# indrajeetadityaroy9/vit-bias-aware-structural-distillation

Measured on AMD Instinct MI355X. Metric: images/sec BASD train step, DeiT-T student / ViT-B teacher bs=256, higher is better.
Workload: dtype bf16

## Files before the change

### vit-bias-aware-structural-distillation_amd/csrc/attention.hip

```cpp
#include "basd_frag.h"

namespace basd {

__device__ __forceinline__ unsigned short f32_to_bf16_rne(float f) {
  unsigned int u = __float_as_uint(f);
  u += 0x7fffu + ((u >> 16) & 1u);
  return (unsigned short)(u >> 16);
}

template <int CTRL> __device__ __forceinline__ float at_dpp_add(float v) {
  return v + __int_as_float(__builtin_amdgcn_update_dpp(0, __float_as_int(v), CTRL, 0xF, 0xF, true));
}

template <int NKT, int AT_HD, bool QMEAN = false>
__global__ __launch_bounds__(256) __attribute__((amdgpu_waves_per_eu(2, 2))) void attention_fwd_kernel(const unsigned short* __restrict__ qkv, int T, int H,
                                                            float scale, unsigned short* __restrict__ out,
                                                            float* __restrict__ importance, float* __restrict__ lse) {
  constexpr int NKS = (NKT + 1) / 2;
  constexpr int KROWS = 32 * NKS;
  constexpr int NDS = (AT_HD + 31) / 32;
  constexpr int NDT = AT_HD / 16;
  constexpr int NCH = AT_HD / 8;
  constexpr int NCHP = NDS * 4;
  constexpr int AT_LD = NDS * 32 + 8;
  extern __shared__ __align__(16) unsigned short sm[];
  unsigned short* Ks = sm;
  unsigned short* Vs = Ks + KROWS * AT_LD;
  unsigned short* Os = Vs + KROWS * AT_LD;
  const int tid = threadIdx.x, lane = tid & 63, wave = tid >> 6;
  const int li = lane & 15, g = lane >> 4;
  const int b = blockIdx.x / H, h = blockIdx.x - b * H;
  const size_t row = (size_t)3 * H * AT_HD;
  const unsigned short* base = qkv + (size_t)b * T * row + (size_t)h * AT_HD;

  constexpr int NLD = (KROWS * NCHP + 255) / 256;
  uint4 kreg[NLD], vreg[NLD];
#pragma unroll
  for (int i = 0; i < NLD; ++i) {
    const int idx = tid + 256 * i;
    const int r = idx / NCHP, c8 = idx - r * NCHP;
    kreg[i] = make_uint4(0, 0, 0, 0);
    vreg[i] = make_uint4(0, 0, 0, 0);
    if (r < T && c8 < NCH) {
      const unsigned short* p = base + (size_t)r * row + c8 * 8;
      kreg[i] = *reinterpret_cast<const uint4*>(p + (size_t)H * AT_HD);
      vreg[i] = *reinterpret_cast<const uint4*>(p + (size_t)2 * H * AT_HD);
    }
  }
#pragma unroll
  for (int i = 0; i < NLD; ++i) {
    const int idx = tid + 256 * i;
    const int r = idx / NCHP, c8 = idx - r * NCHP;
    if (idx < KROWS * NCHP) {
      *reinterpret_cast<uint4*>(Ks + r * AT_LD + c8 * 8) = kreg[i];
      *reinterpret_cast<uint4*>(Vs + r * AT_LD + c8 * 8) = vreg[i];
    }
  }
  __syncthreads();

  const float sl2 = scale * 1.4426950408889634f;
  const int nqt = (T + 15) >> 4;
  const int full_tiles = T >> 4;
  unsigned short* Ow = Os + wave * 16 * AT_LD;
  auto load_q = [&](int qt_, uint4 (&dst)[NDS]) {
#pragma unroll
    for (int ks = 0; ks < NDS; ++ks) {
      dst[ks] = make_uint4(0, 0, 0, 0);
      if (qt_ < nqt && qt_ * 16 + li < T && 32 * ks + 8 * g < AT_HD)
        dst[ks] = *reinterpret_cast<const uint4*>(base + (size_t)(qt_ * 16 + li) * row + 32 * ks + 8 * g);
    }
  };
  uint4 qnext[NDS];
  load_q(wave, qnext);
  float csum[QMEAN ? NKT : 1][4];
#pragma unroll
  for (int kt = 0; kt < (QMEAN ? NKT : 1); ++kt)
#pragma unroll
    for (int r = 0; r < 4; ++r) csum[kt][r] = 0.f;
  for (int qt = wave; qt < nqt; qt += 4) {
    const int q0 = qt * 16;
    bf16x8 qf[NDS];
#pragma unroll
    for (int ks = 0; ks < NDS; ++ks) qf[ks] = *reinterpret_cast<bf16x8*>(&qnext[ks]);
    load_q(qt + 4, qnext);
    f32x4 s[NKT];
#pragma unroll
    for (int kt = 0; kt < NKT; ++kt) {
      f32x4 acc = {0.f, 0.f, 0.f, 0.f};
#pragma unroll
      for (int ks = 0; ks < NDS; ++ks) {
        const uint4 kk = *reinterpret_cast<const uint4*>(Ks + (16 * kt + li) * AT_LD + 32 * ks + 8 * g);
        acc = __builtin_amdgcn_mfma_f32_16x16x32_bf16(*reinterpret_cast<const bf16x8*>(&kk), qf[ks], acc, 0, 0, 0);
      }
      s[kt] = acc;
      if ((kt & 3) == 3) __builtin_amdgcn_sched_barrier(0);
    }
    if (!QMEAN && importance != nullptr && qt == 0) {
      float lr[NKT][4];
      float tmx = -3.0e38f;
#pragma unroll
      for (int kt = 0; kt < NKT; ++kt)
#pragma unroll
        for (int r = 0; r < 4; r += 2) {
          const unsigned int w = pack_bf16(s[kt][r], s[kt][r + 1]);
          lr[kt][r] = __uint_as_float(w << 16) * scale;
          lr[kt][r + 1] = __uint_as_float(w & 0xffff0000u) * scale;
          if (kt >= full_tiles) {
            if (16 * kt + 4 * g + r >= T) lr[kt][r] = -3.0e38f;
            if (16 * kt + 4 * g + r + 1 >= T) lr[kt][r + 1] = -3.0e38f;
          }
          tmx = fmaxf(tmx, fmaxf(lr[kt][r], lr[kt][r + 1]));
        }
      tmx = fmaxf(tmx, __shfl_xor(tmx, 16, 64));
      tmx = fmaxf(tmx, __shfl_xor(tmx, 32, 64));
      float tsum = 0.f;
#pragma unroll
      for (int kt = 0; kt < NKT; ++kt)
#pragma unroll
        for (int r = 0; r < 4; ++r) {
          lr[kt][r] = __builtin_amdgcn_exp2f((lr[kt][r] - tmx) * 1.4426950408889634f);
          tsum += lr[kt][r];
        }
      tsum += __shfl_xor(tsum, 16, 64);
      tsum += __shfl_xor(tsum, 32, 64);
      if (li == 0) {
        const float tinv = 1.f / (tsum * (float)H);
#pragma unroll
        for (int kt = 0; kt < NKT; ++kt)
#pragma unroll
          for (int r = 0; r < 4; ++r) {
            const int key = 16 * kt + 4 * g + r;
            if (key >= 1 && (kt < full_tiles || key < T))
              importance[((size_t)b * H + h) * (T - 1) + key - 1] = lr[kt][r] * tinv;
          }
      }
    }
    float mx = -3.0e38f;
#pragma unroll
    for (int kt = 0; kt < NKT; ++kt)
#pragma unroll
      for (int r = 0; r < 4; ++r) {
        if (kt >= full_tiles && 16 * kt + 4 * g + r >= T) s[kt][r] = -3.0e38f;
        mx = fmaxf(mx, s[kt][r]);
      }
    mx = fmaxf(mx, __shfl_xor(mx, 16, 64));
    mx = fmaxf(mx, __shfl_xor(mx, 32, 64));
    float sum = 0.f;
#pragma unroll
    for (int kt = 0; kt < NKT; ++kt)
#pragma unroll
      for (int r = 0; r < 4; ++r) {
        const float p = __builtin_amdgcn_exp2f((s[kt][r] - mx) * sl2);
        s[kt][r] = p;
        sum += p;
      }
    sum += __shfl_xor(sum, 16, 64);
    sum += __shfl_xor(sum, 32, 64);
    const float inv = 1.f / sum;
    if constexpr (QMEAN) {
      const float qinv = (q0 + li < T) ? inv : 0.f;
#pragma unroll
      for (int kt = 0; kt < NKT; ++kt)
#pragma unroll
        for (int r = 0; r < 4; ++r) csum[kt][r] = fmaf(s[kt][r], qinv, csum[kt][r]);
    }
    if (lse != nullptr && g == 0 && q0 + li < T) lse[((size_t)b * H + h) * T + q0 + li] = fmaf(mx, scale, __logf(sum));
    f32x4 o[NDT];
#pragma unroll
    for (int dt = 0; dt < NDT; ++dt) o[dt] = (f32x4){0.f, 0.f, 0.f, 0.f};
#pragma unroll
    for (int ks = 0; ks < NKS; ++ks) {
      const int K1 = (2 * ks + 1 < NKT) ? 2 * ks + 1 : 0;
      uint4 pw;
      pw.x = pack_bf16(s[2 * ks][0] * inv, s[2 * ks][1] * inv);
      pw.y = pack_bf16(s[2 * ks][2] * inv, s[2 * ks][3] * inv);
      pw.z = (2 * ks + 1 < NKT) ? pack_bf16(s[K1][0] * inv, s[K1][1] * inv) : 0u;
      pw.w = (2 * ks + 1 < NKT) ? pack_bf16(s[K1][2] * inv, s[K1][3] * inv) : 0u;
      const bf16x8 pa = *reinterpret_cast<const bf16x8*>(&pw);
      const int qq = li >> 2, pp = li & 3;
#pragma unroll
      for (int dt = 0; dt < NDT; ++dt) {
        const unsigned short* a0 = Vs + (32 * ks + 4 * g + qq) * AT_LD + 16 * dt + 4 * pp;
        const v4s lo = __builtin_amdgcn_ds_read_tr16_b64_v4i16((lds_v4s*)a0);
        const v4s hi = __builtin_amdgcn_ds_read_tr16_b64_v4i16((lds_v4s*)(a0 + 16 * AT_LD));
        const bf16x8 vb = {lo[0], lo[1], lo[2], lo[3], hi[0], hi[1], hi[2], hi[3]};
        o[dt] = __builtin_amdgcn_mfma_f32_16x16x32_bf16(pa, vb, o[dt], 0, 0, 0);
      }
    }
#pragma unroll
    for (int dt = 0; dt < NDT; ++dt)
#pragma unroll
      for (int r = 0; r < 4; r += 2) {
        const unsigned int w = pack_bf16(o[dt][r], o[dt][r + 1]);
        Ow[(4 * g + r) * AT_LD + 16 * dt + li] = (unsigned short)(w & 0xffffu);
        Ow[(4 * g + r + 1) * AT_LD + 16 * dt + li] = (unsigned short)(w >> 16);
      }
    __builtin_amdgcn_s_waitcnt(0xc07f);
#pragma unroll
    for (int c = 0; c < (16 * NCH + 63) / 64; ++c) {
      const int idx = lane + 64 * c, r = idx / NCH, c8 = idx - r * NCH;
      if (idx < 16 * NCH && q0 + r < T) {
        const uint4 v = *reinterpret_cast<const uint4*>(Ow + r * AT_LD + c8 * 8);
        *reinterpret_cast<uint4*>(out + ((size_t)(b * T + q0 + r) * H + h) * AT_HD + c8 * 8) = v;
      }
    }
    __builtin_amdgcn_s_waitcnt(0xc07f);
  }
  if constexpr (QMEAN) {
    float* cw = reinterpret_cast<float*>(Os) + wave * (16 * AT_LD / 2);
#pragma unroll
    for (int kt = 0; kt < NKT; ++kt)
#pragma unroll
      for (int r = 0; r < 4; ++r) {
        float v = csum[kt][r];
        v = at_dpp_add<0xB1>(v);
        v = at_dpp_add<0x4E>(v);
        v = at_dpp_add<0x124>(v);
        v = at_dpp_add<0x128>(v);
        if (li == 0) cw[16 * kt + 4 * g + r] = v;
      }
    __syncthreads();
    const float* c0 = reinterpret_cast<const float*>(Os);
    const float norm = 1.f / ((float)H * (float)T);
    for (int key = tid; key < T; key += 256) {
      float v = 0.f;
#pragma unroll
      for (int w = 0; w < 4; ++w) v += c0[w * (16 * AT_LD / 2) + key];
      importance[((size_t)b * H + h) * T + key] = v * norm;
    }
  }
}

template <int NKT, int HD, bool QMEAN = false>
static void launch_attention(const void* qkv, int B, int T, int H, float scale, void* out, float* importance,
                             float* lse, hipStream_t st) {
  constexpr int KROWS = 32 * ((NKT + 1) / 2);
  constexpr int LD = (HD + 31) / 32 * 32 + 8;
  const size_t lds = ((size_t)2 * KROWS * LD + 4 * 16 * LD) * sizeof(unsigned short);
  static_assert(8 * LD >= KROWS, "the output staging tile of a wave holds its query-mean column sums");
  allow_full_lds((const void*)attention_fwd_kernel<NKT, HD, QMEAN>);
  hipLaunchKernelGGL((attention_fwd_kernel<NKT, HD, QMEAN>), dim3(B * H), dim3(256), lds, st, (const unsigned short*)qkv, T, H,
                     scale, (unsigned short*)out, importance, lse);
}

}

extern "C" int basd_attention_fwd_bf16(const void* qkv, int B, int T, int H, int hd, float scale, void* out,
                                       float* importance, float* lse, void* stream) {
  using namespace basd;
  if (B <= 0) return BASD_OK;
  if ((hd != 64 && hd != 80) || T < 1 || T > 272 || H < 1)
    return fail(BASD_ERR_SHAPE, "attention_fwd: T=%d H=%d hd=%d unsupported (hd 64 | 80, T <= 272)", T, H, hd);
  if (importance != nullptr && T < 2) return fail(BASD_ERR_SHAPE, "attention_fwd: importance needs T >= 2");
  hipStream_t st = (hipStream_t)stream;
  if (hd == 64) {
    if (T <= 64) launch_attention<4, 64>(qkv, B, T, H, scale, out, importance, lse, st);
    else if (T <= 208) launch_attention<13, 64>(qkv, B, T, H, scale, out, importance, lse, st);
    else launch_attention<17, 64>(qkv, B, T, H, scale, out, importance, lse, st);
  } else {
    if (T <= 208) launch_attention<13, 80>(qkv, B, T, H, scale, out, importance, lse, st);
    else launch_attention<17, 80>(qkv, B, T, H, scale, out, importance, lse, st);
  }
  return check_launch("attention_fwd");
}

extern "C" int basd_attention_fwd_qmean_bf16(const void* qkv, int B, int T, int H, int hd, float scale, void* out,
                                             float* importance, void* stream) {
  using namespace basd;
  if (B <= 0) return BASD_OK;
  if ((hd != 64 && hd != 80) || T < 1 || T > 272 || H < 1)
    return fail(BASD_ERR_SHAPE, "attention_fwd_qmean: T=%d H=%d hd=%d unsupported (hd 64 | 80, T <= 272)", T, H, hd);
  if (importance == nullptr) return fail(BASD_ERR_SHAPE, "attention_fwd_qmean: importance is required");
  hipStream_t st = (hipStream_t)stream;
  if (hd == 64) {
    if (T <= 64) launch_attention<4, 64, true>(qkv, B, T, H, scale, out, importance, nullptr, st);
    else if (T <= 208) launch_attention<13, 64, true>(qkv, B, T, H, scale, out, importance, nullptr, st);
    else launch_attention<17, 64, true>(qkv, B, T, H, scale, out, importance, nullptr, st);
  } else {
    if (T <= 208) launch_attention<13, 80, true>(qkv, B, T, H, scale, out, importance, nullptr, st);
    else launch_attention<17, 80, true>(qkv, B, T, H, scale, out, importance, nullptr, st);
  }
  return check_launch("attention_fwd_qmean");
}
```

Before: 8000.

## Make attention kernel persistent over heads with prefetched K/V and variable wave count

Turns the attention forward kernel into a persistent kernel. Each workgroup walks a contiguous run of (batch, head) pairs, with the grid sized to compute units times resident slots, and prefetches the next head's K/V and Q into registers while it computes the current head. It also uses 8 waves when the K/V LDS footprint is large, and adds a T<=96 specialization for hd=64. The aim is to hide global load latency and cut launch and tail imbalance, at the cost of more register pressure, an extra barrier per head, and clamped loads instead of guarded ones.

```diff
diff --git a/vit-bias-aware-structural-distillation_amd/csrc/attention.hip b/vit-bias-aware-structural-distillation_amd/csrc/attention.hip
--- a/vit-bias-aware-structural-distillation_amd/csrc/attention.hip
+++ b/vit-bias-aware-structural-distillation_amd/csrc/attention.hip
@@ -1,3 +1,4 @@
+#include <type_traits>
 #include "basd_frag.h"
 
 namespace basd {
@@ -12,10 +13,11 @@
   return v + __int_as_float(__builtin_amdgcn_update_dpp(0, __float_as_int(v), CTRL, 0xF, 0xF, true));
 }
 
-template <int NKT, int AT_HD, bool QMEAN = false>
-__global__ __launch_bounds__(256) __attribute__((amdgpu_waves_per_eu(2, 2))) void attention_fwd_kernel(const unsigned short* __restrict__ qkv, int T, int H,
+template <int NKT, int AT_HD, int NW, bool WALK, bool QMEAN = false>
+__global__ __launch_bounds__(64 * NW) __attribute__((amdgpu_waves_per_eu(2, 2))) void attention_fwd_kernel(const unsigned short* __restrict__ qkv, int T, int H,
                                                             float scale, unsigned short* __restrict__ out,
-                                                            float* __restrict__ importance, float* __restrict__ lse) {
+                                                            float* __restrict__ importance, float* __restrict__ lse,
+                                                            int heads, int run, int longer) {
   constexpr int NKS = (NKT + 1) / 2;
   constexpr int KROWS = 32 * NKS;
   constexpr int NDS = (AT_HD + 31) / 32;
@@ -27,208 +29,273 @@
   unsigned short* Ks = sm;
   unsigned short* Vs = Ks + KROWS * AT_LD;
   unsigned short* Os = Vs + KROWS * AT_LD;
-  const int tid = threadIdx.x, lane = tid & 63, wave = tid >> 6;
+  const int tid = threadIdx.x, lane = tid & 63;
+  const int wave = __builtin_amdgcn_readfirstlane(tid >> 6);
   const int li = lane & 15, g = lane >> 4;
-  const int b = blockIdx.x / H, h = blockIdx.x - b * H;
   const size_t row = (size_t)3 * H * AT_HD;
-  const unsigned short* base = qkv + (size_t)b * T * row + (size_t)h * AT_HD;
-
-  constexpr int NLD = (KROWS * NCHP + 255) / 256;
+  const int wg = blockIdx.x;
+  const int head0 = WALK ? wg * run + (wg < longer ? wg : longer) : wg;
+  const int nrun = WALK ? run + (wg < longer ? 1 : 0) : 1;
+  auto head_base = [&](int head) {
+    const int b_ = head / H;
+    return qkv + (size_t)b_ * T * row + (size_t)(head - b_ * H) * AT_HD;
+  };
+
+  constexpr int NLD = (KROWS * NCHP + 64 * NW - 1) / (64 * NW);
   uint4 kreg[NLD], vreg[NLD];
-#pragma unroll
-  for (int i = 0; i < NLD; ++i) {
-    const int idx = tid + 256 * i;
-    const int r = idx / NCHP, c8 = idx - r * NCHP;
-    kreg[i] = make_uint4(0, 0, 0, 0);
-    vreg[i] = make_uint4(0, 0, 0, 0);
-    if (r < T && c8 < NCH) {
-      const unsigned short* p = base + (size_t)r * row + c8 * 8;
+  auto load_kv = [&](const unsigned short* base_, const int live) {
+#pragma unroll
+    for (int i = 0; i < NLD; ++i) {
+      const int idx = tid + 64 * NW * i;
+      const int r = idx / NCHP, c8 = idx - r * NCHP;
+      const int rc = r < T ? r : T - 1, cc = c8 < NCH ? c8 : NCH - 1;
+      const unsigned short* p = base_ + (size_t)live * ((size_t)rc * row + cc * 8);
       kreg[i] = *reinterpret_cast<const uint4*>(p + (size_t)H * AT_HD);
       vreg[i] = *reinterpret_cast<const uint4*>(p + (size_t)2 * H * AT_HD);
     }
-  }
-#pragma unroll
-  for (int i = 0; i < NLD; ++i) {
-    const int idx = tid + 256 * i;
-    const int r = idx / NCHP, c8 = idx - r * NCHP;
-    if (idx < KROWS * NCHP) {
-      *reinterpret_cast<uint4*>(Ks + r * AT_LD + c8 * 8) = kreg[i];
-      *reinterpret_cast<uint4*>(Vs + r * AT_LD + c8 * 8) = vreg[i];
-    }
-  }
-  __syncthreads();
+  };
 
   const float sl2 = scale * 1.4426950408889634f;
   const int nqt = (T + 15) >> 4;
   const int full_tiles = T >> 4;
   unsigned short* Ow = Os + wave * 16 * AT_LD;
-  auto load_q = [&](int qt_, uint4 (&dst)[NDS]) {
+  auto load_q = [&](const unsigned short* base_, const int qt_, const int live, uint4 (&dst)[NDS]) {
+    const int qr = qt_ * 16 + li < T ? qt_ * 16 + li : T - 1;
 #pragma unroll
     for (int ks = 0; ks < NDS; ++ks) {
-      dst[ks] = make_uint4(0, 0, 0, 0);
-      if (qt_ < nqt && qt_ * 16 + li < T && 32 * ks + 8 * g < AT_HD)
-        dst[ks] = *reinterpret_cast<const uint4*>(base + (size_t)(qt_ * 16 + li) * row + 32 * ks + 8 * g);
+      const int col = 32 * ks + 8 * g < AT_HD ? 32 * ks + 8 * g : AT_HD - 8;
+      dst[ks] = *reinterpret_cast<const uint4*>(base_ + (size_t)live * ((size_t)qr * row + col));
     }
   };
-  uint4 qnext[NDS];
-  load_q(wave, qnext);
-  float csum[QMEAN ? NKT : 1][4];
-#pragma unroll
-  for (int kt = 0; kt < (QMEAN ? NKT : 1); ++kt)
-#pragma unroll
-    for (int r = 0; r < 4; ++r) csum[kt][r] = 0.f;
-  for (int qt = wave; qt < nqt; qt += 4) {
-    const int q0 = qt * 16;
-    bf16x8 qf[NDS];
-#pragma unroll
-    for (int ks = 0; ks < NDS; ++ks) qf[ks] = *reinterpret_cast<bf16x8*>(&qnext[ks]);
-    load_q(qt + 4, qnext);
-    f32x4 s[NKT];
-#pragma unroll
-    for (int kt = 0; kt < NKT; ++kt) {
-      f32x4 acc = {0.f, 0.f, 0.f, 0.f};
-#pragma unroll
-      for (int ks = 0; ks < NDS; ++ks) {
-        const uint4 kk = *reinterpret_cast<const uint4*>(Ks + (16 * kt + li) * AT_LD + 32 * ks + 8 * g);
-        acc = __builtin_amdgcn_mfma_f32_16x16x32_bf16(*reinterpret_cast<const bf16x8*>(&kk), qf[ks], acc, 0, 0, 0);
-      }
-      s[kt] = acc;
-      if ((kt & 3) == 3) __builtin_amdgcn_sched_barrier(0);
-    }
-    if (!QMEAN && importance != nullptr && qt == 0) {
-      float lr[NKT][4];
-      float tmx = -3.0e38f;
+  auto q_ready = [&](const uint4 (&src)[NDS], const int qt_, const int live, uint4 (&dst)[NDS]) {
+#pragma unroll
+    for (int ks = 0; ks < NDS; ++ks)
+      dst[ks] = (live && qt_ * 16 + li < T && 32 * ks + 8 * g < AT_HD) ? src[ks] : make_uint4(0, 0, 0, 0);
+  };
+  const unsigned short* base = head_base(head0);
+  uint4 qnext[NDS], qcur[NDS];
+  load_q(base, wave, wave < nqt, qnext);
+  load_kv(base, 1);
+  q_ready(qnext, wave, wave < nqt, qcur);
+  for (int j = 0; j < nrun; ++j) {
+    const int head = head0 + j;
+    const int b = head / H, h = head - b * H;
+    const int first = (wave + j) % NW;
+    const int more = j + 1 < nrun;
+    const unsigned short* nbase = more ? head_base(head + 1) : base;
+    const int nfirst = (wave + j + 1) % NW;
+    if (j > 0) __syncthreads();
+#pragma unroll
+    for (int i = 0; i < NLD; ++i) {
+      const int idx = tid + 64 * NW * i;
+      const int r = idx / NCHP, c8 = idx - r * NCHP;
+      if (idx < KROWS * NCHP) {
+        const bool data = r < T && c8 < NCH;
+        *reinterpret_cast<uint4*>(Ks + r * AT_LD + c8 * 8) = data ? kreg[i] : make_uint4(0, 0, 0, 0);
+        *reinterpret_cast<uint4*>(Vs + r * AT_LD + c8 * 8) = data ? vreg[i] : make_uint4(0, 0, 0, 0);
+      }
+    }
+    __syncthreads();
+    float csum[QMEAN ? NKT : 1][4];
+#pragma unroll
+    for (int kt = 0; kt < (QMEAN ? NKT : 1); ++kt)
+#pragma unroll
+      for (int r = 0; r < 4; ++r) csum[kt][r] = 0.f;
+    auto tile = [&](const int qt, auto ord_c) __attribute__((always_inline)) {
+      constexpr int ORD = decltype(ord_c)::value;
+      constexpr bool TAP = ORD == 0;
+      const int q0 = qt * 16;
+      bf16x8 qf[NDS];
+#pragma unroll
+      for (int ks = 0; ks < NDS; ++ks) qf[ks] = *reinterpret_cast<bf16x8*>(&qcur[ks]);
+      const bool here = qt + NW < nqt;
+      const int nqt_ = here ? qt + NW : nfirst, nlive = here || (more && nfirst < nqt);
+      load_q(here ? base : nbase, nqt_, nlive, qnext);
+      if (WALK && ORD == 1) load_kv(nbase, more);
+      f32x4 s[NKT];
+#pragma unroll
+      for (int kt = 0; kt < NKT; ++kt) {
+        f32x4 acc = {0.f, 0.f, 0.f, 0.f};
+#pragma unroll
+        for (int ks = 0; ks < NDS; ++ks) {
+          const uint4 kk = *reinterpret_cast<const uint4*>(Ks + (16 * kt + li) * AT_LD + 32 * ks + 8 * g);
+          acc = __builtin_amdgcn_mfma_f32_16x16x32_bf16(*reinterpret_cast<const bf16x8*>(&kk), qf[ks], acc, 0, 0, 0);
+        }
+        s[kt] = acc;
+        if ((kt & 3) == 3) __builtin_amdgcn_sched_barrier(0);
+      }
+      if (TAP && !QMEAN && importance != nullptr && qt == 0) {
+        float lr[NKT][4];
+        float tmx = -3.0e38f;
+#pragma unroll
+        for (int kt = 0; kt < NKT; ++kt)
+#pragma unroll
+          for (int r = 0; r < 4; r += 2) {
+            const unsigned int w = pack_bf16(s[kt][r], s[kt][r + 1]);
+            lr[kt][r] = __uint_as_float(w << 16) * scale;
+            lr[kt][r + 1] = __uint_as_float(w & 0xffff0000u) * scale;
+            if (kt >= full_tiles) {
+              if (16 * kt + 4 * g + r >= T) lr[kt][r] = -3.0e38f;
+              if (16 * kt + 4 * g + r + 1 >= T) lr[kt][r + 1] = -3.0e38f;
+            }
+            tmx = fmaxf(tmx, fmaxf(lr[kt][r], lr[kt][r + 1]));
+          }
+        tmx = fmaxf(tmx, __shfl_xor(tmx, 16, 64));
+        tmx = fmaxf(tmx, __shfl_xor(tmx, 32, 64));
+        float tsum = 0.f;
+#pragma unroll
+        for (int kt = 0; kt < NKT; ++kt)
+#pragma unroll
+          for (int r = 0; r < 4; ++r) {
+            lr[kt][r] = __builtin_amdgcn_exp2f((lr[kt][r] - tmx) * 1.4426950408889634f);
+            tsum += lr[kt][r];
+          }
+        tsum += __shfl_xor(tsum, 16, 64);
+        tsum += __shfl_xor(tsum, 32, 64);
+        if (li == 0) {
+          const float tinv = 1.f / (tsum * (float)H);
+#pragma unroll
+          for (int kt = 0; kt < NKT; ++kt)
+#pragma unroll
+            for (int r = 0; r < 4; ++r) {
+              const int key = 16 * kt + 4 * g + r;
+              if (key >= 1 && (kt < full_tiles || key < T))
+                importance[((size_t)b * H + h) * (T - 1) + key - 1] = lr[kt][r] * tinv;
+            }
+        }
+      }
+      float mx = -3.0e38f;
 #pragma unroll
       for (int kt = 0; kt < NKT; ++kt)
 #pragma unroll
+        for (int r = 0; r < 4; ++r) {
+          if (kt >= full_tiles && 16 * kt + 4 * g + r >= T) s[kt][r] = -3.0e38f;
+          mx = fmaxf(mx, s[kt][r]);
+        }
+      mx = fmaxf(mx, __shfl_xor(mx, 16, 64));
+      mx = fmaxf(mx, __shfl_xor(mx, 32, 64));
+      float sum = 0.f;
+#pragma unroll
+      for (int kt = 0; kt < NKT; ++kt)
+#pragma unroll
+        for (int r = 0; r < 4; ++r) {
+          const float p = __builtin_amdgcn_exp2f((s[kt][r] - mx) * sl2);
+          s[kt][r] = p;
+          sum += p;
+        }
+      sum += __shfl_xor(sum, 16, 64);
+      sum += __shfl_xor(sum, 32, 64);
+      const float inv = 1.f / sum;
+      if constexpr (QMEAN) {
+        const float qinv = (q0 + li < T) ? inv : 0.f;
+#pragma unroll
+        for (int kt = 0; kt < NKT; ++kt)
+#pragma unroll
+          for (int r = 0; r < 4; ++r) csum[kt][r] = fmaf(s[kt][r], qinv, csum[kt][r]);
+      }
+      if (lse != nullptr && g == 0 && q0 + li < T) lse[((size_t)b * H + h) * T + q0 + li] = fmaf(mx, scale, __logf(sum));
+      f32x4 o[NDT];
+#pragma unroll
+      for (int dt = 0; dt < NDT; ++dt) o[dt] = (f32x4){0.f, 0.f, 0.f, 0.f};
+#pragma unroll
+      for (int ks = 0; ks < NKS; ++ks) {
+        const int K1 = (2 * ks + 1 < NKT) ? 2 * ks + 1 : 0;
+        uint4 pw;
+        pw.x = pack_bf16(s[2 * ks][0] * inv, s[2 * ks][1] * inv);
+        pw.y = pack_bf16(s[2 * ks][2] * inv, s[2 * ks][3] * inv);
+        pw.z = (2 * ks + 1 < NKT) ? pack_bf16(s[K1][0] * inv, s[K1][1] * inv) : 0u;
+        pw.w = (2 * ks + 1 < NKT) ? pack_bf16(s[K1][2] * inv, s[K1][3] * inv) : 0u;
+        const bf16x8 pa = *reinterpret_cast<const bf16x8*>(&pw);
+        const int qq = li >> 2, pp = li & 3;
+#pragma unroll
+        for (int dt = 0; dt < NDT; ++dt) {
+          const unsigned short* a0 = Vs + (32 * ks + 4 * g + qq) * AT_LD + 16 * dt + 4 * pp;
+          const v4s lo = __builtin_amdgcn_ds_read_tr16_b64_v4i16((lds_v4s*)a0);
+          const v4s hi = __builtin_amdgcn_ds_read_tr16_b64_v4i16((lds_v4s*)(a0 + 16 * AT_LD));
+          const bf16x8 vb = {lo[0], lo[1], lo[2], lo[3], hi[0], hi[1], hi[2], hi[3]};
+          o[dt] = __builtin_amdgcn_mfma_f32_16x16x32_bf16(pa, vb, o[dt], 0, 0, 0);
+        }
+      }
+#pragma unroll
+      for (int dt = 0; dt < NDT; ++dt)
+#pragma unroll
         for (int r = 0; r < 4; r += 2) {
-          const unsigned int w = pack_bf16(s[kt][r], s[kt][r + 1]);
-          lr[kt][r] = __uint_as_float(w << 16) * scale;
-          lr[kt][r + 1] = __uint_as_float(w & 0xffff0000u) * scale;
-          if (kt >= full_tiles) {
-            if (16 * kt + 4 * g + r >= T) lr[kt][r] = -3.0e38f;
-            if (16 * kt + 4 * g + r + 1 >= T) lr[kt][r + 1] = -3.0e38f;
-          }
-          tmx = fmaxf(tmx, fmaxf(lr[kt][r], lr[kt][r + 1]));
-        }
-      tmx = fmaxf(tmx, __shfl_xor(tmx, 16, 64));
-      tmx = fmaxf(tmx, __shfl_xor(tmx, 32, 64));
-      float tsum = 0.f;
+          const unsigned int w = pack_bf16(o[dt][r], o[dt][r + 1]);
+          Ow[(4 * g + r) * AT_LD + 16 * dt + li] = (unsigned short)(w & 0xffffu);
+          Ow[(4 * g + r + 1) * AT_LD + 16 * dt + li] = (unsigned short)(w >> 16);
+        }
+      __builtin_amdgcn_s_waitcnt(0xc07f);
+      if (nlive) q_ready(qnext, nqt_, nlive, qcur);
+#pragma unroll
+      for (int c = 0; c < (16 * NCH + 63) / 64; ++c) {
+        const int idx = lane + 64 * c, r = idx / NCH, c8 = idx - r * NCH;
+        if (idx < 16 * NCH && q0 + r < T) {
+          const uint4 v = *reinterpret_cast<const uint4*>(Ow + r * AT_LD + c8 * 8);
+          *reinterpret_cast<uint4*>(out + ((size_t)(b * T + q0 + r) * H + h) * AT_HD + c8 * 8) = v;
+        }
+      }
+      __builtin_amdgcn_s_waitcnt(0xc07f);
+    };
+    if (first < nqt) {
+      tile(first, std::integral_constant<int, 0>{});
+    } else {
+      load_q(nbase, nfirst, more && nfirst < nqt, qnext);
+      q_ready(qnext, nfirst, more && nfirst < nqt, qcur);
+    }
+    if (first + NW < nqt) tile(first + NW, std::integral_constant<int, 1>{});
+    else if (WALK) load_kv(nbase, more);
+    for (int qt = first + 2 * NW; qt < nqt; qt += NW) tile(qt, std::integral_constant<int, 2>{});
+    if constexpr (QMEAN) {
+      float* cw = reinterpret_cast<float*>(Os) + wave * (16 * AT_LD / 2);
 #pragma unroll
       for (int kt = 0; kt < NKT; ++kt)
 #pragma unroll
         for (int r = 0; r < 4; ++r) {
-          lr[kt][r] = __builtin_amdgcn_exp2f((lr[kt][r] - tmx) * 1.4426950408889634f);
-          tsum += lr[kt][r];
-        }
-      tsum += __shfl_xor(tsum, 16, 64);
-      tsum += __shfl_xor(tsum, 32, 64);
-      if (li == 0) {
-        const float tinv = 1.f / (tsum * (float)H);
-#pragma unroll
-        for (int kt = 0; kt < NKT; ++kt)
-#pragma unroll
-          for (int r = 0; r < 4; ++r) {
-            const int key = 16 * kt + 4 * g + r;
-            if (key >= 1 && (kt < full_tiles || key < T))
-              importance[((size_t)b * H + h) * (T - 1) + key - 1] = lr[kt][r] * tinv;
-          }
-      }
-    }
-    float mx = -3.0e38f;
-#pragma unroll
-    for (int kt = 0; kt < NKT; ++kt)
-#pragma unroll
-      for (int r = 0; r < 4; ++r) {
-        if (kt >= full_tiles && 16 * kt + 4 * g + r >= T) s[kt][r] = -3.0e38f;
-        mx = fmaxf(mx, s[kt][r]);
-      }
-    mx = fmaxf(mx, __shfl_xor(mx, 16, 64));
-    mx = fmaxf(mx, __shfl_xor(mx, 32, 64));
-    float sum = 0.f;
-#pragma unroll
-    for (int kt = 0; kt < NKT; ++kt)
-#pragma unroll
-      for (int r = 0; r < 4; ++r) {
-        const float p = __builtin_amdgcn_exp2f((s[kt][r] - mx) * sl2);
-        s[kt][r] = p;
-        sum += p;
-      }
-    sum += __shfl_xor(sum, 16, 64);
-    sum += __shfl_xor(sum, 32, 64);
-    const float inv = 1.f / sum;
-    if constexpr (QMEAN) {
-      const float qinv = (q0 + li < T) ? inv : 0.f;
-#pragma unroll
-      for (int kt = 0; kt < NKT; ++kt)
-#pragma unroll
-        for (int r = 0; r < 4; ++r) csum[kt][r] = fmaf(s[kt][r], qinv, csum[kt][r]);
-    }
-    if (lse != nullptr && g == 0 && q0 + li < T) lse[((size_t)b * H + h) * T + q0 + li] = fmaf(mx, scale, __logf(sum));
-    f32x4 o[NDT];
-#pragma unroll
-    for (int dt = 0; dt < NDT; ++dt) o[dt] = (f32x4){0.f, 0.f, 0.f, 0.f};
-#pragma unroll
-    for (int ks = 0; ks < NKS; ++ks) {
-      const int K1 = (2 * ks + 1 < NKT) ? 2 * ks + 1 : 0;
-      uint4 pw;
-      pw.x = pack_bf16(s[2 * ks][0] * inv, s[2 * ks][1] * inv);
-      pw.y = pack_bf16(s[2 * ks][2] * inv, s[2 * ks][3] * inv);
-      pw.z = (2 * ks + 1 < NKT) ? pack_bf16(s[K1][0] * inv, s[K1][1] * inv) : 0u;
-      pw.w = (2 * ks + 1 < NKT) ? pack_bf16(s[K1][2] * inv, s[K1][3] * inv) : 0u;
-      const bf16x8 pa = *reinterpret_cast<const bf16x8*>(&pw);
-      const int qq = li >> 2, pp = li & 3;
-#pragma unroll
-      for (int dt = 0; dt < NDT; ++dt) {
-        const unsigned short* a0 = Vs + (32 * ks + 4 * g + qq) * AT_LD + 16 * dt + 4 * pp;
-        const v4s lo = __builtin_amdgcn_ds_read_tr16_b64_v4i16((lds_v4s*)a0);
-        const v4s hi = __builtin_amdgcn_ds_read_tr16_b64_v4i16((lds_v4s*)(a0 + 16 * AT_LD));
-        const bf16x8 vb = {lo[0], lo[1], lo[2], lo[3], hi[0], hi[1], hi[2], hi[3]};
-        o[dt] = __builtin_amdgcn_mfma_f32_16x16x32_bf16(pa, vb, o[dt], 0, 0, 0);
-      }
-    }
-#pragma unroll
-    for (int dt = 0; dt < NDT; ++dt)
-#pragma unroll
-      for (int r = 0; r < 4; r += 2) {
-        const unsigned int w = pack_bf16(o[dt][r], o[dt][r + 1]);
-        Ow[(4 * g + r) * AT_LD + 16 * dt + li] = (unsigned short)(w & 0xffffu);
-        Ow[(4 * g + r + 1) * AT_LD + 16 * dt + li] = (unsigned short)(w >> 16);
-      }
-    __builtin_amdgcn_s_waitcnt(0xc07f);
-#pragma unroll
-    for (int c = 0; c < (16 * NCH + 63) / 64; ++c) {
-      const int idx = lane + 64 * c, r = idx / NCH, c8 = idx - r * NCH;
-      if (idx < 16 * NCH && q0 + r < T) {
-        const uint4 v = *reinterpret_cast<const uint4*>(Ow + r * AT_LD + c8 * 8);
-        *reinterpret_cast<uint4*>(out + ((size_t)(b * T + q0 + r) * H + h) * AT_HD + c8 * 8) = v;
-      }
-    }
-    __builtin_amdgcn_s_waitcnt(0xc07f);
+          float v = csum[kt][r];
+          v = at_dpp_add<0xB1>(v);
+          v = at_dpp_add<0x4E>(v);
+          v = at_dpp_add<0x124>(v);
+          v = at_dpp_add<0x128>(v);
+          if (li == 0) cw[16 * kt + 4 * g + r] = v;
+        }
+      __syncthreads();
+      const float* c0 = reinterpret_cast<const float*>(Os);
+      const float norm = 1.f / ((float)H * (float)T);
+      for (int key = tid; key < T; key += 64 * NW) {
+        float v = 0.f;
+#pragma unroll
+        for (int w = 0; w < NW; ++w) v += c0[w * (16 * AT_LD / 2) + key];
+        importance[((size_t)b * H + h) * T + key] = v * norm;
+      }
+    }
+    base = nbase;
   }
-  if constexpr (QMEAN) {
-    float* cw = reinterpret_cast<float*>(Os) + wave * (16 * AT_LD / 2);
-#pragma unroll
-    for (int kt = 0; kt < NKT; ++kt)
-#pragma unroll
-      for (int r = 0; r < 4; ++r) {
-        float v = csum[kt][r];
-        v = at_dpp_add<0xB1>(v);
-        v = at_dpp_add<0x4E>(v);
-        v = at_dpp_add<0x124>(v);
-        v = at_dpp_add<0x128>(v);
-        if (li == 0) cw[16 * kt + 4 * g + r] = v;
-      }
-    __syncthreads();
-    const float* c0 = reinterpret_cast<const float*>(Os);
-    const float norm = 1.f / ((float)H * (float)T);
-    for (int key = tid; key < T; key += 256) {
-      float v = 0.f;
-#pragma unroll
-      for (int w = 0; w < 4; ++w) v += c0[w * (16 * AT_LD / 2) + key];
-      importance[((size_t)b * H + h) * T + key] = v * norm;
-    }
+}
+
+static int compute_units() {
+  static thread_local int cus = 0;
+  if (cus == 0) {
+    int dev = 0, n = 0;
+    if (hipGetDevice(&dev) != hipSuccess ||
+        hipDeviceGetAttribute(&n, hipDeviceAttributeMultiprocessorCount, dev) != hipSuccess || n < 1)
+      n = 256;
+    cus = n;
   }
+  return cus;
+}
+
+static int walk_grid(int heads, size_t lds) {
+  const int slots = compute_units() * (lds <= 80 * 1024 ? 2 : 1);
+  return heads < slots ? heads : slots;
+}
+
+template <int NKT, int HD, int NW, bool WALK, bool QMEAN>
+static void launch_attention_grid(const void* qkv, int T, int H, float scale, void* out, float* importance, float* lse,
+                                  int heads, int grid, size_t lds, hipStream_t st) {
+  allow_full_lds((const void*)attention_fwd_kernel<NKT, HD, NW, WALK, QMEAN>);
+  hipLaunchKernelGGL((attention_fwd_kernel<NKT, HD, NW, WALK, QMEAN>), dim3(grid), dim3(64 * NW), lds, st,
+                     (const unsigned short*)qkv, T, H, scale, (unsigned short*)out, importance, lse, heads, heads / grid,
+                     heads % grid);
 }
 
 template <int NKT, int HD, bool QMEAN = false>
@@ -236,11 +303,15 @@
                              float* lse, hipStream_t st) {
   constexpr int KROWS = 32 * ((NKT + 1) / 2);
   constexpr int LD = (HD + 31) / 32 * 32 + 8;
-  const size_t lds = ((size_t)2 * KROWS * LD + 4 * 16 * LD) * sizeof(unsigned short);
+  constexpr int NW = ((size_t)2 * KROWS * LD * sizeof(unsigned short) > 72 * 1024) ? 8 : 4;
+  constexpr bool WALK = !QMEAN && !(NKT == 17 && HD == 80);
+  const size_t lds = ((size_t)2 * KROWS * LD + NW * 16 * LD) * sizeof(unsigned short);
   static_assert(8 * LD >= KROWS, "the output staging tile of a wave holds its query-mean column sums");
-  allow_full_lds((const void*)attention_fwd_kernel<NKT, HD, QMEAN>);
-  hipLaunchKernelGGL((attention_fwd_kernel<NKT, HD, QMEAN>), dim3(B * H), dim3(256), lds, st, (const unsigned short*)qkv, T, H,
-                     scale, (unsigned short*)out, importance, lse);
+  const int heads = B * H, grid = WALK ? walk_grid(heads, lds) : heads;
+  if (WALK && grid < heads)
+    launch_attention_grid<NKT, HD, NW, WALK, QMEAN>(qkv, T, H, scale, out, importance, lse, heads, grid, lds, st);
+  else
+    launch_attention_grid<NKT, HD, NW, false, QMEAN>(qkv, T, H, scale, out, importance, lse, heads, heads, lds, st);
 }
 
 }
@@ -255,6 +326,7 @@
   hipStream_t st = (hipStream_t)stream;
   if (hd == 64) {
     if (T <= 64) launch_attention<4, 64>(qkv, B, T, H, scale, out, importance, lse, st);
+    else if (T <= 96) launch_attention<6, 64>(qkv, B, T, H, scale, out, importance, lse, st);
     else if (T <= 208) launch_attention<13, 64>(qkv, B, T, H, scale, out, importance, lse, st);
     else launch_attention<17, 64>(qkv, B, T, H, scale, out, importance, lse, st);
   } else {
@@ -274,6 +346,7 @@
   hipStream_t st = (hipStream_t)stream;
   if (hd == 64) {
     if (T <= 64) launch_attention<4, 64, true>(qkv, B, T, H, scale, out, importance, nullptr, st);
+    else if (T <= 96) launch_attention<6, 64, true>(qkv, B, T, H, scale, out, importance, nullptr, st);
     else if (T <= 208) launch_attention<13, 64, true>(qkv, B, T, H, scale, out, importance, nullptr, st);
     else launch_attention<17, 64, true>(qkv, B, T, H, scale, out, importance, nullptr, st);
   } else {
```

Result: no change. 7937 (-0.8%).
